# Shuijing725/CrowdNav_Prediction_AttnGraph

Measured on AMD Instinct MI355X. Metric: env-steps/sec (sim+policy fwd) at 20 humans, higher is better.
Workload: dtype f32 (big GEMMs as bf16x3 split-precision MFMA, fp32 accumulate); 1 GPU; BASELINE configs[1]: CrowdSimVarNum-v0, 20 humans, 4096 parallel envs per GPU, HH+HR attention on, policy forward + ORCA sim step + auto-reset per step; envs_per_gpu=4096, humans=20, parallelism=dp1 (envs sharded, no rollout collective), policy_init=orthogonal, torch.manual_seed(425), sampled_actions=True, side_stream_tail=inline, dephase_steps=240

## Files before the change

### crowdnav_prediction_attngraph_amd/_abi.py

```python
import ctypes as C
import os

_PKG = os.path.dirname(os.path.abspath(__file__))
LIB_PATH = os.environ.get("CN_HIP_LIB") or os.path.join(_PKG, "libcrowdnav_hip.so")

CN_MAX_HUMANS = 64
ABI_VERSION = 407
PROF_KERNELS, PROF_SLOT_WORDS = 8, 2048
PROF_KERNEL_IDS = {"env_step": 0, "orca_lane": 1, "hh_fused": 2, "rn_fused": 3, "orca_lp3": 4, "env_pregen": 5, "row_plan": 6, "other": 7}
ENV_KINDS = {"CrowdSimVarNum-v0": 0, "CrowdSimPred-v0": 1, "CrowdSimPredRealGST-v0": 2, "CrowdSimVarNumCollect-v0": 3}
GSTD_MODES = {None: 0, "train": 1, "val": 2, "test": 2}
GSTD_FRAME_ORDER, GSTD_DUPLICATE_ID, GSTD_TOO_MANY_PEDS = 1, 2, 4
INFO_NOTHING, INFO_TIMEOUT, INFO_COLLISION, INFO_REACHGOAL, INFO_DANGER = range(5)


class CnError(RuntimeError):
    pass


class EnvConfig(C.Structure):
    _fields_ = [
        ("human_num", C.c_int32), ("predict_steps", C.c_int32), ("env_kind", C.c_int32),
        ("randomize_attributes", C.c_int32), ("random_goal_changing", C.c_int32),
        ("end_goal_changing", C.c_int32), ("sort_humans", C.c_int32), ("phase", C.c_int32),
# ... 191 lines not shown

class SrnnEdgeGrads(C.Structure):
    _fields_ = [(name, C.c_void_p) for name, _ in SRNN_EDGE_KEYS]


class PpoBatch(C.Structure):
    _fields_ = [(n, C.c_int) for n in ("T", "N", "E", "H", "D")] + [(n, C.c_void_p) for n in PPO_BATCH_TENSORS]


class PpoHyper(C.Structure):
    _fields_ = [("clip_param", C.c_float), ("value_loss_coef", C.c_float), ("entropy_coef", C.c_float), ("use_clipped_value_loss", C.c_int)]


ABI_SYMBOLS = [
    "cn_last_error", "cn_version", "cn_device_count", "cn_env_config_default", "cn_env_create", "cn_env_destroy",
    "cn_env_obs_width", "cn_row_plan_words", "cn_env_set_pregen_budget", "cn_env_set_tail_deferral", "cn_env_launch_tail", "cn_policy_set_post_hh_hook", "cn_env_reset", "cn_env_step", "cn_env_join", "cn_env_get_state", "cn_env_get_human_actions", "cn_env_get_danger_min_dist", "cn_env_get_human_counts", "cn_env_set_case_counters", "cn_env_snapshot_bytes", "cn_env_save", "cn_env_load", "cn_orca_solve",
    "cn_policy_create", "cn_policy_create_sized", "cn_policy_destroy", "cn_policy_set_weights", "cn_policy_act", "cn_policy_get_value",
    "cn_policy_get_taps", "cn_policy_set_gemm_mode", "cn_policy_set_self_attention", "cn_obs_compact_visible", "cn_policy_set_taps", "cn_policy_set_profiling", "cn_policy_get_profile",
    "cn_policy_get_profile_samples", "cn_policy_reset_profile", "cn_prof_set_stamps", "cn_prof_next_step", "cn_hh_block_workspace_bytes", "cn_hh_block_fwd", "cn_rn_seq_workspace_floats", "cn_rn_seq_fwd_workspace_floats", "cn_rn_seq_fwd", "cn_rn_seq_bwd", "cn_rn_seq_workspace_floats_sized", "cn_rn_seq_fwd_workspace_floats_sized", "cn_rn_seq_fwd_sized", "cn_rn_seq_bwd_sized", "cn_gru_seq_fwd_sized", "cn_gru_seq_bwd_sized", "cn_hh_attention_workspace_ints", "cn_hh_attention_fwd", "cn_hh_attention_bwd", "cn_hr_attention_fwd", "cn_hr_attention_bwd", "cn_gru_seq_fwd", "cn_gru_seq_bwd", "cn_embed0_fwd", "cn_embed0_bwd",
    "cn_split_bf16", "cn_split_bf16_padded", "cn_linear_fwd", "cn_linear_fwd_act", "cn_linear_wgrad_splits", "cn_linear_wgrad", "cn_small_mm", "cn_gst_create", "cn_gst_create_horizon", "cn_gst_pred_steps", "cn_gst_destroy", "cn_gst_set_weights", "cn_gst_predict",
    "cn_gst_wrapper_reset", "cn_gst_wrapper_step", "cn_gst_wrapper_set_interval", "cn_gst_wrapper_history_len", "cn_gst_wrapper_save", "cn_gst_wrapper_load", "cn_gae", "cn_adv_stats", "cn_adv_normalize", "cn_episode_stats_update", "cn_eval_state_words", "cn_eval_accumulate",
    "cn_ppo_loss_workspace_doubles", "cn_ppo_loss_fwd", "cn_ppo_loss_bwd", "cn_adam_workspace_doubles", "cn_adam_clip_step",
    "cn_ppo_minibatch_max_rows", "cn_ppo_minibatch_workspace_bytes", "cn_ppo_row_totals", "cn_ppo_minibatch_step",
    "cn_gst_train_workspace_bytes", "cn_gst_train_step", "cn_gst_eval_workspace_bytes", "cn_gst_eval_step",
    "cn_gst_train_workspace_bytes_horizon", "cn_gst_train_step_horizon", "cn_gst_eval_workspace_bytes_horizon", "cn_gst_eval_step_horizon",
    "cn_gst_data_frames_horizon", "cn_gst_data_count_horizon", "cn_gst_data_fill_horizon", "cn_gst_gather_batch_horizon",
    "cn_env_get_visibility", "cn_render_scenes",
    "cn_env_trace_append", "cn_trace_metrics", "cn_render_trajectories",
    "cn_gst_data_frames", "cn_gst_data_count", "cn_gst_data_fill", "cn_gst_gather_batch",
    "cn_srnn_create", "cn_srnn_destroy", "cn_srnn_set_weights", "cn_srnn_act", "cn_srnn_get_value", "cn_srnn_get_taps", "cn_srnn_set_gemm_mode",
    "cn_srnn_seq_workspace_bytes", "cn_srnn_seq_fwd", "cn_srnn_seq_bwd",
# ... 20 lines not shown
                          % (LIB_PATH, L.cn_version(), ABI_VERSION))
        L.cn_env_config_default.argtypes = [C.POINTER(EnvConfig)]
        L.cn_env_config_default.restype = None
        L.cn_env_create.argtypes = [C.POINTER(EnvConfig), i32, i64, i64, C.POINTER(vp)]
        L.cn_env_destroy.argtypes = [vp]
        L.cn_env_obs_width.argtypes = [C.POINTER(EnvConfig)]
        L.cn_env_reset.argtypes = [vp, C.POINTER(Obs), vp]
        L.cn_env_step.argtypes = [vp, vp, C.POINTER(Obs), vp, vp, vp, vp, vp, vp, vp]
        L.cn_env_join.argtypes = [vp, vp]
        L.cn_env_set_pregen_budget.argtypes = [vp, C.c_int64]
        L.cn_env_set_tail_deferral.argtypes = [vp, i32]
        L.cn_env_launch_tail.argtypes = [vp, vp]
        L.cn_policy_set_post_hh_hook.argtypes = [vp, vp, vp]
        L.cn_row_plan_words.restype = C.c_int64
        L.cn_row_plan_words.argtypes = [C.c_int]
        L.cn_env_get_state.argtypes = [vp, vp, vp, vp]
        L.cn_env_get_danger_min_dist.argtypes = [vp, vp, vp]
        L.cn_env_set_case_counters.argtypes = [vp, vp, vp]
        L.cn_env_get_human_counts.argtypes = [vp, vp, vp]
        L.cn_env_get_human_actions.argtypes = [vp, vp, vp]
        L.cn_env_get_visibility.argtypes = [vp, vp, vp]
        L.cn_render_scenes.argtypes = [i32, i32, vp, vp, vp, vp, vp, vp, vp, i32, f32, f32, i32, f32, vp, vp]
        L.cn_env_trace_append.argtypes = [vp, vp, vp, i32, vp, vp, vp, vp, vp]
        L.cn_trace_metrics.argtypes = [i32, i32, i32, vp, vp, vp, f64, f64, vp, vp]
        L.cn_render_trajectories.argtypes = [i32, i32, i32, vp, vp, vp, vp, i32, i32, f32, vp, vp]
        L.cn_env_snapshot_bytes.argtypes = [vp]
        L.cn_env_snapshot_bytes.restype = i64
        L.cn_env_save.argtypes = [vp, vp, vp]
        L.cn_env_load.argtypes = [vp, vp, vp]
        L.cn_orca_solve.argtypes = [i32, i32, vp, vp, f32, i32, f32, f32, vp, vp]
# ... 174 lines not shown
```

### crowdnav_prediction_attngraph_amd/csrc/env_sim.hip

```cpp
#include "common.h"
#include "env_dev.h"
#include "env_profile.h"
#include "det_math.h"
#include "orca.h"
#include "mt19937.h"
#include "episode.h"

#include <hip/hip_ext.h>
#include <cmath>
#include <cstdio>
#include <cstdlib>
#include <cstring>
#include <new>
#include <type_traits>

namespace {

__global__ __launch_bounds__(64) void env_reset_kernel(EnvDev s, cn_obs ob, int with_obs)
{
    const int lane = threadIdx.x;
    const int e = blockIdx.x;
    Rng R{MT_N, false};
    Robot rb{};
    Lane h{};
// ... 833 lines not shown
    b->pregen_ticks = 4000;
    b->lp3_blocks = lp3_grid(num_envs * HM);
    *out = b;
    return CN_OK;
}

extern "C" int cn_env_set_pregen_budget(cn_env_batch *env, int64_t ticks_10ns)
{
    CN_REQUIRE(env && ticks_10ns >= 0, "cn_env_set_pregen_budget: null handle or negative budget");
    env->pregen_ticks = ticks_10ns;
    return CN_OK;
}

extern "C" int64_t cn_row_plan_words(int num_envs) { return num_envs > 0 ? (int64_t)rp_words(num_envs) : 0; }

extern "C" int cn_env_destroy(cn_env_batch *env)
{
    if (!env) return CN_OK;
    (void)hipStreamSynchronize(env->side);
    if (env->side2) { (void)hipStreamSynchronize(env->side2); (void)hipStreamDestroy(env->side2); }
    if (env->ev_pg) (void)hipEventDestroy(env->ev_pg);
    (void)hipEventDestroy(env->ev_state); (void)hipEventDestroy(env->ev_orca); (void)hipEventDestroy(env->ev_pre); (void)hipStreamDestroy(env->side);
    if (env->blob) CN_HIP(hipFree(env->blob));
    delete env;
    return CN_OK;
}

static int check_obs(const cn_obs *obs)
{
    CN_REQUIRE(obs && obs->robot_node && obs->temporal_edges && obs->spatial_edges && obs->detected_human_num,
// ... 217 lines not shown
```

### crowdnav_prediction_attngraph_amd/csrc/orca.h

```cpp
#pragma once
#include "env_dev.h"
#include "det_math.h"

namespace {

struct LpLine { float px, py, dx, dy; };

__device__ __forceinline__ bool wv_any(bool p) { return __ballot(p) != 0ull; }

__device__ __forceinline__ bool lp1_wave(const LpLine &L, uint64_t valid, int i, float ipx, float ipy, float idx, float idy,
                                         float radius, float optx, float opty, bool dirOpt, int lane, float &rx, float &ry)
{
    const float dotProduct = ipx * idx + ipy * idy;
    const float discriminant = dotProduct * dotProduct + radius * radius - (ipx * ipx + ipy * ipy);
    if (discriminant < 0.0f) return false;
    const float sq = sqrtf(discriminant);
    float tLeft = -dotProduct - sq;
    float tRight = -dotProduct + sq;
    const bool mine = lane < i && ((valid >> lane) & 1ull);
    const float denominator = idx * L.dy - idy * L.dx;
    const float numerator = L.dx * (ipy - L.py) - L.dy * (ipx - L.px);
    const bool parallel = fabsf(denominator) <= RVO_EPS;
    const bool pfail = mine && parallel && numerator < 0.0f;
    const float t = numerator / denominator;
// ... 390 lines not shown
    if (plan && (int)blockIdx.x < plan_groups) {
        __builtin_amdgcn_s_setprio(3);
        rowplan::build((int)blockIdx.x, plan_groups, s.E, s.H, rp_workgroups(s.E, s.H), plan_det, plan, *reinterpret_cast<rowplan::Lds *>(s_raw), nullptr, s.plan_arrive);
        return;
    }
    const int blk = (int)blockIdx.x - (plan ? plan_groups : 0);
    typedef typename LaneVec<VW>::f vec;
    const int agent = blk * 64 + threadIdx.x;
    const int H = s.H;
    const bool live_lane = agent < s.E * H;
    const int e = live_lane ? agent / H : (blk * 64) / H, i = live_lane ? agent - e * H : 0;
    const int n = crowd_size(s, e);
    const bool active = live_lane && i < n;
    const cn_env_config &c = s.cfg;
    constexpr int NENV = NB == 8 ? 65 : (NB == 20 ? 10 : 5);
    __shared__ double s_px[128], s_py[128], s_vx[128], s_vy[128], s_rad[128], s_rob[NENV][4];
    const double *hum = s.hum + (size_t)e * 8 * H;
    const size_t ei = (size_t)e * H + i;
    double sgx, sgy, svpref, shared_nd_in;
    int sim_valid_in, sim_n_in = 0;
    float sim_nd_in, sim_r_in, sim_ms_in;
    {
        const int a0 = blk * 64;
        const int e0 = a0 / H, e1 = (min(a0 + 63, s.E * H - 1)) / H;
        const int nrows = (e1 - e0 + 1) * H;
        double st[2][5];
#pragma unroll
        for (int it = 0; it < 2; ++it) {
            const int r = threadIdx.x + 64 * it;
            if (r < nrows) {
                const int ee = e0 + r / H, j = r - (r / H) * H;
                const double *hm = s.hum + (size_t)ee * 8 * H;
                st[it][0] = hm[F_PX * H + j]; st[it][1] = hm[F_PY * H + j]; st[it][2] = hm[F_VX * H + j]; st[it][3] = hm[F_VY * H + j];
                st[it][4] = hm[F_RAD * H + j];
            }
        }
        sgx = hum[F_GX * H + i]; sgy = hum[F_GY * H + i]; svpref = hum[F_VPREF * H + i];
        sim_valid_in = s.sim_valid[ei];
        if (s.sim_n) sim_n_in = s.sim_n[ei];
        sim_nd_in = s.sim_nd[ei]; sim_r_in = s.sim_self_radius[ei]; sim_ms_in = s.sim_self_maxspeed[ei];
        shared_nd_in = s.shared_nd[e];
#pragma unroll
        for (int it = 0; it < 2; ++it) {
            const int r = threadIdx.x + 64 * it;
            if (r < nrows) { s_px[r] = st[it][0]; s_py[r] = st[it][1]; s_vx[r] = st[it][2]; s_vy[r] = st[it][3]; s_rad[r] = st[it][4]; }
        }
        if (c.robot_visible)
            for (int q = threadIdx.x; q <= e1 - e0; q += 64) {
                const double *rb = s.rob + (size_t)(e0 + q) * 8;
                s_rob[q][0] = rb[R_PX]; s_rob[q][1] = rb[R_PY]; s_rob[q][2] = rb[R_VX]; s_rob[q][3] = rb[R_VY];
            }
        __syncthreads();
    }
    const int eq = e - (blk * 64) / H, eb = eq * H;
    const double spx = s_px[eb + i], spy = s_py[eb + i], svx = s_vx[eb + i], svy = s_vy[eb + i], srad = s_rad[eb + i];
    const double safety = c.orca_safety_space;
    const bool rv = c.robot_visible != 0;
    const int n_agents = n + (rv ? 1 : 0);
    float nd = 0.0f, self_r = 0.0f, self_ms = 0.0f;
    if (active) {
        const bool rebuild = !sim_valid_in || (s.sim_n && sim_n_in != n_agents);
        if (rebuild) {
            nd = (float)shared_nd_in;
            self_r = (float)(srad + 0.01 + safety);
            self_ms = (float)svpref;
            if (s.sim_seen)
                for (int j = 0; j < n; ++j) s.sim_seen[ei * H + j] = (float)(s_rad[eb + j] + 0.01 + safety);
            s.sim_nd[ei] = nd; s.sim_self_radius[ei] = self_r; s.sim_self_maxspeed[ei] = self_ms; s.sim_valid[ei] = 1;
            if (s.sim_n) s.sim_n[ei] = (uint8_t)n_agents;
        } else {
            nd = sim_nd_in; self_r = sim_r_in; self_ms = sim_ms_in;
        }
    }
    const float fpx = (float)spx, fpy = (float)spy, fvx = (float)svx, fvy = (float)svy;
    vec key, idx;
    int nn = 0;
#pragma unroll 1
    for (int j = 0; j < NB; ++j) {
        const bool isR = rv && j == n;
        const bool cand = active && ((j < n && j != i) || isR);
        const int lj = j < n ? j : 0;
        const double qx = isR ? s_rob[eq][0] : s_px[eb + lj], qy = isR ? s_rob[eq][1] : s_py[eb + lj];
        const bool coincident = (qx == spx) && (qy == spy);
        const float opx = coincident ? 7.0f : (float)qx, opy = coincident ? 7.0f : (float)qy;
        const float ddx0 = fpx - opx, ddy0 = fpy - opy;
        const float dq = ddx0 * ddx0 + ddy0 * ddy0;
        const bool inrange = cand && dq < nd * nd;
        key[j] = inrange ? dq : INFINITY;
        idx[j] = (float)j;
        nn += inrange ? 1 : 0;
    }
#define ORCA_CE(a, b)                                                                                  \
    {                                                                                                  \
        const float ka0 = key[a], kb0 = key[b], ia0 = idx[a], ib0 = idx[b];                             \
        const bool sw = kb0 < ka0 || (kb0 == ka0 && ib0 < ia0);                                         \
        key[a] = sw ? kb0 : ka0; key[b] = sw ? ka0 : kb0; idx[a] = sw ? ib0 : ia0; idx[b] = sw ? ia0 : ib0; \
    }
    if constexpr (NB == 8) { ORCA_SORTNET_8(ORCA_CE) }
    else if constexpr (NB == 20) { ORCA_SORTNET_20(ORCA_CE) }
    else { static_assert(NB == 32, "sorting networks exist for 8, 20 and 32 slots"); ORCA_SORTNET_32(ORCA_CE) }
#undef ORCA_CE
    int nmax = nn;
    for (int off = 32; off >= 1; off >>= 1) nmax = max(nmax, __shfl_xor(nmax, off, 64));
    nmax = __builtin_amdgcn_readfirstlane(nmax);
    const float invTH = 1.0f / (float)c.orca_time_horizon, invDT = 1.0f / (float)c.time_step;
    float4 *const s_line = reinterpret_cast<float4 *>(s_raw);
    const int tid = threadIdx.x;
#pragma unroll 1
    for (int k = 0; k < nmax; ++k) {
        float o_px = 0.0f, o_py = 0.0f, o_dx = 1.0f, o_dy = 0.0f;
        const int j = (int)idx[k];
        if (k < nn) {
            const bool isR = j == n;
            const int lj = isR ? 0 : j;
            const double qx = isR ? s_rob[eq][0] : s_px[eb + lj], qy = isR ? s_rob[eq][1] : s_py[eb + lj];
            const double qvx = isR ? s_rob[eq][2] : s_vx[eb + lj], qvy = isR ? s_rob[eq][3] : s_vy[eb + lj];
            float orad;
            if (isR) orad = (float)(c.robot_radius + 0.01 + safety);
            else if (s.sim_seen) orad = s.sim_seen[ei * H + lj];
            else orad = (float)(s_rad[eb + lj] + 0.01 + safety);
            const bool coincident = (qx == spx) && (qy == spy);
            const float opx = coincident ? 7.0f : (float)qx, opy = coincident ? 7.0f : (float)qy;
            const float ovx = coincident ? 0.0f : (float)qvx, ovy = coincident ? 0.0f : (float)qvy;
            const float rpx = opx - fpx, rpy = opy - fpy;
            const float rvx = fvx - ovx, rvy = fvy - ovy;
            const float distSq = rpx * rpx + rpy * rpy;
            const float cr = self_r + orad;
            const float crSq = cr * cr;
            const bool collide = !(distSq > crSq);
            const float invT = collide ? invDT : invTH;
            const float wx = rvx - invT * rpx, wy = rvy - invT * rpy;
            const float wLenSq = wx * wx + wy * wy;
            const float dot1 = wx * rpx + wy * rpy;
            const bool circle = collide || (dot1 < 0.0f && dot1 * dot1 > crSq * wLenSq);
            const float sq = sqrtf(circle ? wLenSq : distSq - crSq);
            const float inv = 1.0f / (circle ? sq : distSq);
            const float uwx = wx * inv, uwy = wy * inv;
            const float sc = cr * invT - sq;
            const bool left = rpx * wy - rpy * wx > 0.0f;
            const float lgx = left ? (rpx * sq - rpy * cr) * inv : -((rpx * sq + rpy * cr) * inv);
            const float lgy = left ? (rpx * cr + rpy * sq) * inv : -((-rpx * cr + rpy * sq) * inv);
            const float dot2 = rvx * lgx + rvy * lgy;
            const float ldx = circle ? uwy : lgx, ldy = circle ? -uwx : lgy;
            const float ux = circle ? sc * uwx : dot2 * lgx - rvx, uy = circle ? sc * uwy : dot2 * lgy - rvy;
            o_px = fvx + 0.5f * ux; o_py = fvy + 0.5f * uy; o_dx = ldx; o_dy = ldy;
        }
        s_line[k * 64 + tid] = make_float4(o_px, o_py, o_dx, o_dy);
    }
    double gvx = sgx - spx, gvy = sgy - spy;
    const double speed = sqrt(gvx * gvx + gvy * gvy);
    if (speed > 1.0) { gvx = gvx / speed; gvy = gvy / speed; }
    const float optx = (float)gvx, opty = (float)gvy, radius = self_ms;
    float rx, ry;
    if (optx * optx + opty * opty > radius * radius) {
        const float inv = 1.0f / sqrtf(optx * optx + opty * opty);
        rx = radius * (optx * inv); ry = radius * (opty * inv);
    } else {
        rx = optx; ry = opty;
    }
    unsigned *const s_tl = reinterpret_cast<unsigned *>(s_line + (NB - 1) * 64), *const s_tr = s_tl + 64;
    int *const s_pf = reinterpret_cast<int *>(s_tr + 64), *const s_vl = s_pf + 64;
    auto okey = [](float f) { const unsigned u = __float_as_uint(f); return u ^ ((u >> 31) ? 0xffffffffu : 0x80000000u); };
    auto okey_inv = [](unsigned o) { return __uint_as_float(o ^ ((o >> 31) ? 0x80000000u : 0xffffffffu)); };
    bool failed = false;
    int line_fail = 0;
#pragma unroll 1
    for (int li = 0; li < nmax; ++li) {
        const float4 Li = s_line[li * 64 + tid];
        const float ipx = Li.x, ipy = Li.y, idx_ = Li.z, idy = Li.w;
        const bool viol = li < nn && !failed && idx_ * (ipy - ry) - idy * (ipx - rx) > 0.0f;
        const unsigned long long vm = __ballot(viol);
        if (vm == 0ull) continue;
        const float dotProduct = ipx * idx_ + ipy * idy;
        const float discriminant = dotProduct * dotProduct + radius * radius - (ipx * ipx + ipy * ipy);
        bool ok = !(discriminant < 0.0f);
        const float sq = sqrtf(discriminant);
        float tLeft = -dotProduct - sq, tRight = -dotProduct + sq;
        bool pfail = false;
        const int npairs = __popcll(vm) * li;
        if (npairs > 0) {
            if (viol) {
                const int rank = __builtin_amdgcn_mbcnt_hi((unsigned)(vm >> 32), __builtin_amdgcn_mbcnt_lo((unsigned)vm, 0u));
                s_vl[rank] = tid; s_tl[tid] = okey(tLeft); s_tr[tid] = okey(tRight); s_pf[tid] = 0;
            }
            __syncthreads();
            const unsigned inv20 = ((1u << 20) + (unsigned)li - 1u) / (unsigned)li;
#pragma unroll 1
            for (int p0 = 0; p0 < npairs; p0 += 64) {
                const int p = p0 + tid;
                const bool on = p < npairs;
                const int r = on ? (int)(((unsigned)p * inv20) >> 20) : 0;
                const int lj = on ? p - r * li : 0;
                const int a = s_vl[r];
                const float4 A = s_line[li * 64 + a], B = s_line[lj * 64 + a];
                const float denominator = A.z * B.w - A.w * B.z;
                const float numerator = B.z * (A.y - B.y) - B.w * (A.x - B.x);
                const bool parallel = fabsf(denominator) <= RVO_EPS;
                const float t = numerator / denominator;
                if (on) {
                    if (parallel) { if (numerator < 0.0f) s_pf[a] = 1; }
                    else if (denominator >= 0.0f) atomicMin(&s_tr[a], okey(t));
// ... 141 lines not shown
```

### crowdnav_prediction_attngraph_amd/csrc/row_plan.h

```cpp
#pragma once
#include <stdint.h>

#define RP_MAGIC 0x52504c4e
#define RP_TMAX 1024
#define RP_EMAX 4096
#define RP_HMAX 32
#define RP_HDR 8

__host__ __device__ inline int rp_off_rowoff() { return RP_HDR; }
__host__ __device__ inline int rp_off_tcnt(int E) { return RP_HDR + ((E + 1 + 3) & ~3); }
__host__ __device__ inline int rp_off_items(int E) { return rp_off_tcnt(E) + RP_TMAX; }
__host__ __device__ inline int rp_words(int E) { return rp_off_items(E) + RP_TMAX * 64; }
__host__ __device__ inline int rp_workgroups(int E, int H)
{
    long long g = ((long long)E * H + 15) / 16;
    return g > 256 ? 256 : (g < 1 ? 1 : (int)g);
}
__host__ __device__ inline int rp_groups(int E)
{
    if (E <= 0 || (E & 255)) return 1;
    return E >= 2048 ? 8 : (E >= 1024 ? 4 : (E >= 512 ? 2 : 1));
}

#ifdef __HIPCC__
// ... 42 lines not shown
template <int TBP>
__device__ __forceinline__ bool fill(int H, int T, int TB, int rows, int hist, int cstart, int id_base, int32_t *__restrict__ items, int32_t *__restrict__ tcnt,
                                     Lds &lds, long long *tim)
{
    const int ln = threadIdx.x & 63;
    int load[TBP], cnt[TBP];
    bool own[TBP];
#pragma unroll
    for (int j = 0; j < TBP; ++j) { load[j] = 0; cnt[j] = 0; own[j] = j < TB && ln * TB + j < T; }
    const int base = rows / T, extra = rows - base * T;
    int cap0[TBP];
#pragma unroll
    for (int j = 0; j < TBP; ++j) { const int c0 = base + (ln * TB + j < extra ? 1 : 0); cap0[j] = c0 > 63 ? 63 : c0; }
    bool bad = false;
    int rot = 0;
    for (int v = H; v >= 1; --v) {
        const int m = __builtin_amdgcn_readlane(hist, v);
        if (m == 0) continue;
        const int pos0 = __builtin_amdgcn_readlane(cstart, v);
        RP_A0();
        const unsigned inv = ((1u << 20) + (unsigned)v - 1u) / (unsigned)v;
        int placed = 0;
        constexpr int NPASS = 13;
        const int raise[NPASS] = {0, 0, 1, 2, 3, 4, 6, 8, 12, 16, 24, 32, 63};
        for (int pass = 0; pass < NPASS && placed < m; ++pass) {
            const int left = m - placed;
            const int quota = pass == 0 ? (left + T - 1) / T : 64;
            int c[TBP], lc = 0;
#pragma unroll
            for (int j = 0; j < TBP; ++j) {
                int cap = cap0[j] + raise[pass];
                cap = cap > 63 ? 63 : cap;
                int r = own[j] && load[j] < cap ? (int)(((unsigned)(cap - load[j]) * inv) >> 20) : 0;
                r = r < 63 - cnt[j] ? r : 63 - cnt[j];
                r = r < quota ? r : quota;
                c[j] = r; lc += r;
// ... 28 lines not shown
            placed += fit < left ? fit : left;
            RP_A(10);
        }
        if (placed < m) bad = true;
    }
#pragma unroll
    for (int j = 0; j < TBP; ++j)
        if (own[j]) {
            tcnt[ln * TB + j] = cnt[j];
            items[(size_t)(ln * TB + j) * 64 + cnt[j]] = 0;
            if (load[j] > 63) bad = true;
        }
    return __ballot(bad) == 0ull;
}

__device__ __forceinline__ void build(int g, int G, int E, int H, int NW, const float *__restrict__ det, int32_t *__restrict__ plan, Lds &lds, long long *tim = nullptr,
                                      int32_t *arrive = nullptr)
{
    const int ln = threadIdx.x & 63;
    int32_t *hdr = plan, *row_off = plan + rp_off_rowoff(), *tcnt = plan + rp_off_tcnt(E), *items = plan + rp_off_items(E);
    RP_T(0);
    if (ln == 0) hdr[0] = 0;
    if (H > RP_HMAX || E > RP_EMAX || (E & 3)) return;
    const int CH = ((E + 255) >> 8) << 2;
    int mysum = 0;
    {
        int c[64];
#pragma unroll
        for (int q = 0; q < 16; ++q) {
            float4 d = float4{0.f, 0.f, 0.f, 0.f};
            const int e0 = ln * CH + 4 * q;
            if (4 * q < CH && e0 < E) d = *reinterpret_cast<const float4 *>(det + e0);
            const float dd[4] = {d.x, d.y, d.z, d.w};
#pragma unroll
            for (int u = 0; u < 4; ++u) {
                int r = (int)dd[u];
                r = r < 1 ? 1 : (r > H ? H : r);
                c[4 * q + u] = (4 * q < CH && e0 < E) ? r : 0;
            }
        }
#pragma unroll
        for (int i = 0; i < 64; ++i) mysum += c[i];
        const int incl0 = wave_incl_scan(mysum);
        const int LG = 64 / G;
        if (ln / LG == g || G == 1) {
            int run = incl0 - mysum;
#pragma unroll
            for (int q = 0; q < 16; ++q) {
                int4 o;
                o.x = run; run += c[4 * q]; o.y = run; run += c[4 * q + 1]; o.z = run; run += c[4 * q + 2]; o.w = run; run += c[4 * q + 3];
                if (4 * q < CH && ln * CH + 4 * q < E) *reinterpret_cast<int4 *>(row_off + ln * CH + 4 * q) = o;
            }
        }
        mysum = incl0;
    }
    const int total = __builtin_amdgcn_readlane(mysum, 63);
    if (g == 0 && ln == 0) row_off[E] = total;
    int n = (total + 62 * NW - 1) / (62 * NW);
    n = n < 1 ? 1 : n;
    const int Tall = n * NW;
    int e_base = 0, Eg = E, t0 = 0, T = Tall, grows = total;
    if (G > 1) {
        const int LG = 64 / G;
        const int cum0 = g ? __builtin_amdgcn_readlane(mysum, g * LG - 1) : 0, cum1 = __builtin_amdgcn_readlane(mysum, (g + 1) * LG - 1);
        grows = cum1 - cum0;
        t0 = (int)(((long long)cum0 * Tall + total / 2) / total);
        const int t1 = g == G - 1 ? Tall : (int)(((long long)cum1 * Tall + total / 2) / total);
        T = t1 - t0;
        Eg = E / G; e_base = g * Eg;
    }
    bool ok = T >= 1 && Tall <= RP_TMAX;
    int c[64];
    int hist = 0, cstart = 0;
    if (ok) {
        const int CHg = ((Eg + 255) >> 8) << 2;
#pragma unroll
        for (int q = 0; q < 16; ++q) {
            float4 d = float4{0.f, 0.f, 0.f, 0.f};
            const int e0 = ln * CHg + 4 * q;
            const bool in = 4 * q < CHg && e0 < Eg;
            if (in) d = *reinterpret_cast<const float4 *>(det + e_base + e0);
            const float dd[4] = {d.x, d.y, d.z, d.w};
#pragma unroll
            for (int u = 0; u < 4; ++u) {
                int r = (int)dd[u];
                r = r < 1 ? 1 : (r > H ? H : r);
                c[4 * q + u] = in ? r : 0;
            }
        }
        for (int k = ln; k < (H + 1) * 64; k += 64) lds.tbl[k] = 0;
#pragma unroll
        for (int i = 0; i < 64; ++i)
            if (c[i]) __hip_atomic_fetch_add(&lds.tbl[c[i] * 64 + ln], 1, __ATOMIC_RELAXED, __HIP_MEMORY_SCOPE_WORKGROUP);
        RP_T(1);
        {
            int at = 0;
            for (int v = H; v >= 1; --v) {
                const int mine = lds.tbl[v * 64 + ln];
                const int incl = wave_incl_scan(mine);
                lds.tbl[v * 64 + ln] = at + incl - mine;
                const int m = __builtin_amdgcn_readlane(incl, 63);
                if (ln == v) { hist = m; cstart = at; }
                at += m;
            }
        }
        {
            int pos[64];
#pragma unroll
            for (int i = 0; i < 64; ++i)
                pos[i] = c[i] ? __hip_atomic_fetch_add(&lds.tbl[c[i] * 64 + ln], 1, __ATOMIC_RELAXED, __HIP_MEMORY_SCOPE_WORKGROUP) : 0;
#pragma unroll
            for (int i = 0; i < 64; ++i)
                if (c[i]) lds.ids[pos[i]] = (unsigned short)(ln * CHg + i);
        }
        RP_T(2);
        const int TB = (T + 63) >> 6;
        int32_t *it = items + (size_t)t0 * 64, *tc = tcnt + t0;
        if (TB <= 1) ok = fill<1>(H, T, TB, grows, hist, cstart, e_base, it, tc, lds, tim);
        else if (TB <= 2) ok = fill<2>(H, T, TB, grows, hist, cstart, e_base, it, tc, lds, tim);
        else if (TB <= 4) ok = fill<4>(H, T, TB, grows, hist, cstart, e_base, it, tc, lds, tim);
        else if (TB <= 8) ok = fill<8>(H, T, TB, grows, hist, cstart, e_base, it, tc, lds, tim);
        else ok = fill<16>(H, T, TB, grows, hist, cstart, e_base, it, tc, lds, tim);
    }
    RP_T(3);
    __threadfence();
    if (ln == 0) {
        int32_t *ctr = arrive ? arrive : &hdr[7];
        const int old = G > 1 ? atomicAdd(ctr, ok ? 1 : 0x10001) : (ok ? 0 : 0x10000);
        if ((old & 0xffff) == G - 1) {
// ... 15 lines not shown
```

### include/crowdnav_hip.h

```cpp
#ifndef CROWDNAV_HIP_H
#define CROWDNAV_HIP_H

#include <stddef.h>
#include <stdint.h>

#ifdef __cplusplus
extern "C" {
#endif

typedef enum {
    CN_OK = 0,
    CN_ERR_INVALID = -1,
    CN_ERR_HIP = -2,
    CN_ERR_NO_DEVICE = -3,
    CN_ERR_STATE = -4
} cn_status;

enum { CN_ENV_VARNUM = 0, CN_ENV_PRED = 1, CN_ENV_PRED_GST = 2, CN_ENV_COLLECT = 3 };
enum { CN_PHASE_TRAIN = 0, CN_PHASE_VAL = 1, CN_PHASE_TEST = 2 };
enum { CN_INFO_NOTHING = 0, CN_INFO_TIMEOUT = 1, CN_INFO_COLLISION = 2, CN_INFO_REACHGOAL = 3, CN_INFO_DANGER = 4 };

enum { CN_ROBOT_NETWORK = 0, CN_ROBOT_ORCA = 1, CN_ROBOT_SOCIAL_FORCE = 2 };
enum { CN_KIN_HOLONOMIC = 0, CN_KIN_UNICYCLE = 1 };
enum { CN_HUMANS_ORCA = 0, CN_HUMANS_SOCIAL_FORCE = 1 };
// ... 44 lines not shown
typedef struct cn_policy cn_policy;

#define CN_ABI_VERSION 407
const char *cn_last_error(void);
int cn_version(void);
int cn_device_count(void);

void cn_env_config_default(cn_env_config *cfg);
int cn_env_create(const cn_env_config *cfg, int num_envs, int64_t seed, int64_t first_env_index, cn_env_batch **out);
int cn_env_destroy(cn_env_batch *env);
int cn_env_obs_width(const cn_env_config *cfg);
int cn_env_set_pregen_budget(cn_env_batch *env, int64_t ticks_10ns);
int cn_env_set_tail_deferral(cn_env_batch *env, int enabled);
int cn_env_launch_tail(cn_env_batch *env, void *stream);
int64_t cn_row_plan_words(int num_envs);
int cn_env_reset(cn_env_batch *env, const cn_obs *obs, void *stream);
int cn_env_step(cn_env_batch *env, const float *actions, const cn_obs *obs, float *reward, uint8_t *done, uint8_t *info,
                double *ep_return, int32_t *ep_len, float *not_done, void *stream);
int cn_env_join(cn_env_batch *env, void *stream);
int cn_env_get_state(cn_env_batch *env, double *humans, double *robot, void *stream);
int cn_env_get_human_actions(cn_env_batch *env, float *out, void *stream);
int cn_env_get_danger_min_dist(cn_env_batch *env, double *out, void *stream);
int cn_env_get_human_counts(cn_env_batch *env, int32_t *out, void *stream);
int cn_env_get_visibility(cn_env_batch *env, uint8_t *out, void *stream);
int cn_env_trace_append(cn_env_batch *env, const int64_t *active, const int64_t *index, int cap, float *agents, uint8_t *flags, float *goal,
                        int32_t *length, void *stream);
int cn_env_set_case_counters(cn_env_batch *env, const uint64_t *counters, void *stream);

int64_t cn_env_snapshot_bytes(const cn_env_batch *env);
int cn_env_save(cn_env_batch *env, void *dst, void *stream);
// ... 301 lines not shown
```

Measured before the change: 16.75 million env-steps/s.

## Use float LDS staging, packed-key sort and templated row-plan histogram in ORCA

The ORCA lane kernel now stages neighbour position, velocity and inflated radius as float4/float in shared memory instead of five double arrays. The neighbour filter runs a fully unrolled float pass and falls back to the exact double coincidence check only when some lane sees an equal position. The sorting network now compares packed 64-bit (key, index) values. Per-lane reciprocal tables replace integer divisions in the LP and row-plan loops. The row-plan builder reuses prefetched detection counts, sizes its histogram and hand-out loops to the real chunk count, and unrolls the class scan by eight; a standalone row-plan build entry point is also added. Together these aim to cut LDS traffic, double-precision arithmetic, register pressure and serial scan latency, at the risk of subtle numeric or ordering differences.

Result: faster. 16.95 million env-steps/s (median of 6 runs) (+1.2%).

```diff
diff --git a/crowdnav_prediction_attngraph_amd/_abi.py b/crowdnav_prediction_attngraph_amd/_abi.py
--- a/crowdnav_prediction_attngraph_amd/_abi.py
+++ b/crowdnav_prediction_attngraph_amd/_abi.py
@@ -229,7 +229,7 @@
 
 ABI_SYMBOLS = [
     "cn_last_error", "cn_version", "cn_device_count", "cn_env_config_default", "cn_env_create", "cn_env_destroy",
-    "cn_env_obs_width", "cn_row_plan_words", "cn_env_set_pregen_budget", "cn_env_set_tail_deferral", "cn_env_launch_tail", "cn_policy_set_post_hh_hook", "cn_env_reset", "cn_env_step", "cn_env_join", "cn_env_get_state", "cn_env_get_human_actions", "cn_env_get_danger_min_dist", "cn_env_get_human_counts", "cn_env_set_case_counters", "cn_env_snapshot_bytes", "cn_env_save", "cn_env_load", "cn_orca_solve",
+    "cn_env_obs_width", "cn_row_plan_words", "cn_row_plan_build", "cn_env_set_pregen_budget", "cn_env_set_tail_deferral", "cn_env_launch_tail", "cn_policy_set_post_hh_hook", "cn_env_reset", "cn_env_step", "cn_env_join", "cn_env_get_state", "cn_env_get_human_actions", "cn_env_get_danger_min_dist", "cn_env_get_human_counts", "cn_env_set_case_counters", "cn_env_snapshot_bytes", "cn_env_save", "cn_env_load", "cn_orca_solve",
     "cn_policy_create", "cn_policy_create_sized", "cn_policy_destroy", "cn_policy_set_weights", "cn_policy_act", "cn_policy_get_value",
     "cn_policy_get_taps", "cn_policy_set_gemm_mode", "cn_policy_set_self_attention", "cn_obs_compact_visible", "cn_policy_set_taps", "cn_policy_set_profiling", "cn_policy_get_profile",
     "cn_policy_get_profile_samples", "cn_policy_reset_profile", "cn_prof_set_stamps", "cn_prof_next_step", "cn_hh_block_workspace_bytes", "cn_hh_block_fwd", "cn_rn_seq_workspace_floats", "cn_rn_seq_fwd_workspace_floats", "cn_rn_seq_fwd", "cn_rn_seq_bwd", "cn_rn_seq_workspace_floats_sized", "cn_rn_seq_fwd_workspace_floats_sized", "cn_rn_seq_fwd_sized", "cn_rn_seq_bwd_sized", "cn_gru_seq_fwd_sized", "cn_gru_seq_bwd_sized", "cn_hh_attention_workspace_ints", "cn_hh_attention_fwd", "cn_hh_attention_bwd", "cn_hr_attention_fwd", "cn_hr_attention_bwd", "cn_gru_seq_fwd", "cn_gru_seq_bwd", "cn_embed0_fwd", "cn_embed0_bwd",
@@ -280,6 +280,7 @@
         L.cn_policy_set_post_hh_hook.argtypes = [vp, vp, vp]
         L.cn_row_plan_words.restype = C.c_int64
         L.cn_row_plan_words.argtypes = [C.c_int]
+        L.cn_row_plan_build.argtypes = [i32, i32, vp, vp, vp]
         L.cn_env_get_state.argtypes = [vp, vp, vp, vp]
         L.cn_env_get_danger_min_dist.argtypes = [vp, vp, vp]
         L.cn_env_set_case_counters.argtypes = [vp, vp, vp]
diff --git a/crowdnav_prediction_attngraph_amd/csrc/env_sim.hip b/crowdnav_prediction_attngraph_amd/csrc/env_sim.hip
--- a/crowdnav_prediction_attngraph_amd/csrc/env_sim.hip
+++ b/crowdnav_prediction_attngraph_amd/csrc/env_sim.hip
@@ -871,6 +871,25 @@
 
 extern "C" int64_t cn_row_plan_words(int num_envs) { return num_envs > 0 ? (int64_t)rp_words(num_envs) : 0; }
 
+__global__ __launch_bounds__(64) void row_plan_kernel(int E, int H, const float *det, int32_t *plan)
+{
+    __shared__ rowplan::Lds lds;
+    rowplan::build((int)blockIdx.x, (int)gridDim.x, E, H, rp_workgroups(E, H), det, plan, lds);
+}
+
+extern "C" int cn_row_plan_build(int num_envs, int rows, const float *detected_human_num, int32_t *row_plan, void *stream)
+{
+    if (int rc = cn_require_device()) return rc;
+    CN_REQUIRE(num_envs > 0 && rows >= 1 && detected_human_num && row_plan, "cn_row_plan_build: null argument or empty batch");
+    CN_REQUIRE((((uintptr_t)detected_human_num | (uintptr_t)row_plan) & 15u) == 0, "cn_row_plan_build: both buffers must be 16-byte aligned");
+    hipStream_t st = (hipStream_t)stream;
+    CN_HIP(hipMemsetAsync(row_plan, 0, RP_HDR * sizeof(int32_t), st));
+    if (num_envs > RP_EMAX) return CN_OK;
+    hipLaunchKernelGGL(row_plan_kernel, dim3(rp_groups(num_envs)), dim3(64), 0, st, num_envs, rows, detected_human_num, row_plan);
+    CN_CHECK_LAUNCH();
+    return CN_OK;
+}
+
 extern "C" int cn_env_destroy(cn_env_batch *env)
 {
     if (!env) return CN_OK;
diff --git a/crowdnav_prediction_attngraph_amd/csrc/orca.h b/crowdnav_prediction_attngraph_amd/csrc/orca.h
--- a/crowdnav_prediction_attngraph_amd/csrc/orca.h
+++ b/crowdnav_prediction_attngraph_amd/csrc/orca.h
@@ -1,6 +1,7 @@
 #pragma once
 #include "env_dev.h"
 #include "det_math.h"
+#include <type_traits>
 
 namespace {
 
@@ -428,9 +429,12 @@
     const bool active = live_lane && i < n;
     const cn_env_config &c = s.cfg;
     constexpr int NENV = NB == 8 ? 65 : (NB == 20 ? 10 : 5);
-    __shared__ double s_px[128], s_py[128], s_vx[128], s_vy[128], s_rad[128], s_rob[NENV][4];
+    __shared__ double s_px[128], s_py[128], s_rob[NENV][2];
+    __shared__ float4 s_f4[128], s_frob[NENV];
+    __shared__ float s_fr[128];
     const double *hum = s.hum + (size_t)e * 8 * H;
     const size_t ei = (size_t)e * H + i;
+    const double safety = c.orca_safety_space;
     double sgx, sgy, svpref, shared_nd_in;
     int sim_valid_in, sim_n_in = 0;
     float sim_nd_in, sim_r_in, sim_ms_in;
@@ -457,18 +461,24 @@
 #pragma unroll
         for (int it = 0; it < 2; ++it) {
             const int r = threadIdx.x + 64 * it;
-            if (r < nrows) { s_px[r] = st[it][0]; s_py[r] = st[it][1]; s_vx[r] = st[it][2]; s_vy[r] = st[it][3]; s_rad[r] = st[it][4]; }
+            if (r < nrows) {
+                s_px[r] = st[it][0]; s_py[r] = st[it][1];
+                s_f4[r] = make_float4((float)st[it][0], (float)st[it][1], (float)st[it][2], (float)st[it][3]);
+                s_fr[r] = (float)(st[it][4] + 0.01 + safety);
+            }
         }
         if (c.robot_visible)
             for (int q = threadIdx.x; q <= e1 - e0; q += 64) {
                 const double *rb = s.rob + (size_t)(e0 + q) * 8;
-                s_rob[q][0] = rb[R_PX]; s_rob[q][1] = rb[R_PY]; s_rob[q][2] = rb[R_VX]; s_rob[q][3] = rb[R_VY];
+                const double rx0 = rb[R_PX], ry0 = rb[R_PY], rvx0 = rb[R_VX], rvy0 = rb[R_VY];
+                s_rob[q][0] = rx0; s_rob[q][1] = ry0;
+                s_frob[q] = make_float4((float)rx0, (float)ry0, (float)rvx0, (float)rvy0);
             }
         __syncthreads();
     }
     const int eq = e - (blk * 64) / H, eb = eq * H;
-    const double spx = s_px[eb + i], spy = s_py[eb + i], svx = s_vx[eb + i], svy = s_vy[eb + i], srad = s_rad[eb + i];
-    const double safety = c.orca_safety_space;
+    const double spx = s_px[eb + i], spy = s_py[eb + i];
+    const float4 self4 = s_f4[eb + i];
     const bool rv = c.robot_visible != 0;
     const int n_agents = n + (rv ? 1 : 0);
     float nd = 0.0f, self_r = 0.0f, self_ms = 0.0f;
@@ -476,66 +486,105 @@
         const bool rebuild = !sim_valid_in || (s.sim_n && sim_n_in != n_agents);
         if (rebuild) {
             nd = (float)shared_nd_in;
-            self_r = (float)(srad + 0.01 + safety);
+            self_r = s_fr[eb + i];
             self_ms = (float)svpref;
             if (s.sim_seen)
-                for (int j = 0; j < n; ++j) s.sim_seen[ei * H + j] = (float)(s_rad[eb + j] + 0.01 + safety);
+                for (int j = 0; j < n; ++j) s.sim_seen[ei * H + j] = s_fr[eb + j];
             s.sim_nd[ei] = nd; s.sim_self_radius[ei] = self_r; s.sim_self_maxspeed[ei] = self_ms; s.sim_valid[ei] = 1;
             if (s.sim_n) s.sim_n[ei] = (uint8_t)n_agents;
         } else {
             nd = sim_nd_in; self_r = sim_r_in; self_ms = sim_ms_in;
         }
     }
-    const float fpx = (float)spx, fpy = (float)spy, fvx = (float)svx, fvy = (float)svy;
+    const float fpx = self4.x, fpy = self4.y, fvx = self4.z, fvy = self4.w;
+    float4 rob4 = make_float4(0.0f, 0.0f, 0.0f, 0.0f);
+    if (rv) rob4 = s_frob[eq];
+    const float rob_r = (float)(c.robot_radius + 0.01 + safety);
     vec key, idx;
     int nn = 0;
+    unsigned coin = 0u;
+    {
+        const float ndSq = nd * nd;
+        bool feq = false;
+        auto pass1 = [&](auto with_robot) {
+#pragma unroll
+            for (int j = 0; j < NB; ++j) {
+                float qx = s_f4[eb + j].x, qy = s_f4[eb + j].y;
+                bool cand = active && j < n && j != i;
+                if constexpr (decltype(with_robot)::value) {
+                    const bool isR = j == n;
+                    qx = isR ? rob4.x : qx; qy = isR ? rob4.y : qy;
+                    cand = cand || (active && isR);
+                }
+                feq |= cand & (qx == fpx) & (qy == fpy);
+                const float ddx0 = fpx - qx, ddy0 = fpy - qy;
+                const float dq = ddx0 * ddx0 + ddy0 * ddy0;
+                const bool inrange = cand && dq < ndSq;
+                key[j] = inrange ? dq : INFINITY;
+                nn += inrange ? 1 : 0;
+                if ((j & 3) == 3) __builtin_amdgcn_sched_barrier(0);
+            }
+        };
+        if (rv) pass1(std::true_type{}); else pass1(std::false_type{});
+        if (__ballot(feq) != 0ull) {
+            nn = 0;
 #pragma unroll 1
-    for (int j = 0; j < NB; ++j) {
-        const bool isR = rv && j == n;
-        const bool cand = active && ((j < n && j != i) || isR);
-        const int lj = j < n ? j : 0;
-        const double qx = isR ? s_rob[eq][0] : s_px[eb + lj], qy = isR ? s_rob[eq][1] : s_py[eb + lj];
-        const bool coincident = (qx == spx) && (qy == spy);
-        const float opx = coincident ? 7.0f : (float)qx, opy = coincident ? 7.0f : (float)qy;
-        const float ddx0 = fpx - opx, ddy0 = fpy - opy;
-        const float dq = ddx0 * ddx0 + ddy0 * ddy0;
-        const bool inrange = cand && dq < nd * nd;
-        key[j] = inrange ? dq : INFINITY;
-        idx[j] = (float)j;
-        nn += inrange ? 1 : 0;
-    }
-#define ORCA_CE(a, b)                                                                                  \
-    {                                                                                                  \
-        const float ka0 = key[a], kb0 = key[b], ia0 = idx[a], ib0 = idx[b];                             \
-        const bool sw = kb0 < ka0 || (kb0 == ka0 && ib0 < ia0);                                         \
-        key[a] = sw ? kb0 : ka0; key[b] = sw ? ka0 : kb0; idx[a] = sw ? ib0 : ia0; idx[b] = sw ? ia0 : ib0; \
-    }
-    if constexpr (NB == 8) { ORCA_SORTNET_8(ORCA_CE) }
-    else if constexpr (NB == 20) { ORCA_SORTNET_20(ORCA_CE) }
-    else { static_assert(NB == 32, "sorting networks exist for 8, 20 and 32 slots"); ORCA_SORTNET_32(ORCA_CE) }
+            for (int j = 0; j < NB; ++j) {
+                const bool isR = rv && j == n;
+                const bool cand = active && ((j < n && j != i) || isR);
+                const int lj = j < n ? j : 0;
+                const double qxd = isR ? s_rob[eq][0] : s_px[eb + lj], qyd = isR ? s_rob[eq][1] : s_py[eb + lj];
+                const float qx = isR ? rob4.x : s_f4[eb + lj].x, qy = isR ? rob4.y : s_f4[eb + lj].y;
+                const bool coincident = (qxd == spx) && (qyd == spy);
+                if (cand && coincident) coin |= 1u << j;
+                const float opx = coincident ? 7.0f : qx, opy = coincident ? 7.0f : qy;
+                const float ddx0 = fpx - opx, ddy0 = fpy - opy;
+                const float dq = ddx0 * ddx0 + ddy0 * ddy0;
+                const bool inrange = cand && dq < ndSq;
+                key[j] = inrange ? dq : INFINITY;
+                nn += inrange ? 1 : 0;
+            }
+        }
+    }
+    const bool any_coin = __ballot(coin != 0u) != 0ull;
+    {
+        unsigned long long kv[NB];
+#pragma unroll
+        for (int j = 0; j < NB; ++j) kv[j] = ((unsigned long long)__float_as_uint(key[j]) << 32) | (unsigned)j;
+#define ORCA_CE(a, b)                                                  \
+    {                                                                  \
+        const unsigned long long ka0 = kv[a], kb0 = kv[b];             \
+        const bool sw = kb0 < ka0;                                     \
+        kv[a] = sw ? kb0 : ka0; kv[b] = sw ? ka0 : kb0;                \
+    }
+        if constexpr (NB == 8) { ORCA_SORTNET_8(ORCA_CE) }
+        else if constexpr (NB == 20) { ORCA_SORTNET_20(ORCA_CE) }
+        else { static_assert(NB == 32, "sorting networks exist for 8, 20 and 32 slots"); ORCA_SORTNET_32(ORCA_CE) }
 #undef ORCA_CE
-    int nmax = nn;
-    for (int off = 32; off >= 1; off >>= 1) nmax = max(nmax, __shfl_xor(nmax, off, 64));
-    nmax = __builtin_amdgcn_readfirstlane(nmax);
-    const float invTH = 1.0f / (float)c.orca_time_horizon, invDT = 1.0f / (float)c.time_step;
+#pragma unroll
+        for (int j = 0; j < NB; ++j) idx[j] = __uint_as_float(held((unsigned)kv[j]));
+    }
+    const int nmax = rowplan::wave_max(nn);
+    const float invTH = held(1.0f / (float)c.orca_time_horizon), invDT = held(1.0f / (float)c.time_step);
     float4 *const s_line = reinterpret_cast<float4 *>(s_raw);
     const int tid = threadIdx.x;
 #pragma unroll 1
     for (int k = 0; k < nmax; ++k) {
         float o_px = 0.0f, o_py = 0.0f, o_dx = 1.0f, o_dy = 0.0f;
-        const int j = (int)idx[k];
+        const int j = (int)__float_as_uint(idx[k]);
         if (k < nn) {
             const bool isR = j == n;
             const int lj = isR ? 0 : j;
-            const double qx = isR ? s_rob[eq][0] : s_px[eb + lj], qy = isR ? s_rob[eq][1] : s_py[eb + lj];
-            const double qvx = isR ? s_rob[eq][2] : s_vx[eb + lj], qvy = isR ? s_rob[eq][3] : s_vy[eb + lj];
+            float4 q = s_f4[eb + lj];
             float orad;
-            if (isR) orad = (float)(c.robot_radius + 0.01 + safety);
-            else if (s.sim_seen) orad = s.sim_seen[ei * H + lj];
-            else orad = (float)(s_rad[eb + lj] + 0.01 + safety);
-            const bool coincident = (qx == spx) && (qy == spy);
-            const float opx = coincident ? 7.0f : (float)qx, opy = coincident ? 7.0f : (float)qy;
-            const float ovx = coincident ? 0.0f : (float)qvx, ovy = coincident ? 0.0f : (float)qvy;
+            if (s.sim_seen) orad = s.sim_seen[ei * H + lj];
+            else orad = held(s_fr[eb + lj]);
+            if (rv) { q.x = isR ? rob4.x : q.x; q.y = isR ? rob4.y : q.y; q.z = isR ? rob4.z : q.z; q.w = isR ? rob4.w : q.w; orad = isR ? rob_r : orad; }
+            if (any_coin) {
+                const bool coincident = (coin >> j) & 1u;
+                q.x = coincident ? 7.0f : q.x; q.y = coincident ? 7.0f : q.y; q.z = coincident ? 0.0f : q.z; q.w = coincident ? 0.0f : q.w;
+            }
+            const float opx = q.x, opy = q.y, ovx = q.z, ovy = q.w;
             const float rpx = opx - fpx, rpy = opy - fpy;
             const float rvx = fvx - ovx, rvy = fvy - ovy;
             const float distSq = rpx * rpx + rpy * rpy;
@@ -546,14 +595,15 @@
             const float wx = rvx - invT * rpx, wy = rvy - invT * rpy;
             const float wLenSq = wx * wx + wy * wy;
             const float dot1 = wx * rpx + wy * rpy;
-            const bool circle = collide || (dot1 < 0.0f && dot1 * dot1 > crSq * wLenSq);
+            const bool circle = collide | ((dot1 < 0.0f) & (dot1 * dot1 > crSq * wLenSq));
             const float sq = sqrtf(circle ? wLenSq : distSq - crSq);
             const float inv = 1.0f / (circle ? sq : distSq);
             const float uwx = wx * inv, uwy = wy * inv;
             const float sc = cr * invT - sq;
             const bool left = rpx * wy - rpy * wx > 0.0f;
-            const float lgx = left ? (rpx * sq - rpy * cr) * inv : -((rpx * sq + rpy * cr) * inv);
-            const float lgy = left ? (rpx * cr + rpy * sq) * inv : -((-rpx * cr + rpy * sq) * inv);
+            const float lxl = (rpx * sq - rpy * cr) * inv, lxr = -((rpx * sq + rpy * cr) * inv);
+            const float lyl = (rpx * cr + rpy * sq) * inv, lyr = -((-rpx * cr + rpy * sq) * inv);
+            const float lgx = left ? lxl : lxr, lgy = left ? lyl : lyr;
             const float dot2 = rvx * lgx + rvy * lgy;
             const float ldx = circle ? uwy : lgx, ldy = circle ? -uwx : lgy;
             const float ux = circle ? sc * uwx : dot2 * lgx - rvx, uy = circle ? sc * uwy : dot2 * lgy - rvy;
@@ -578,6 +628,7 @@
     auto okey_inv = [](unsigned o) { return __uint_as_float(o ^ ((o >> 31) ? 0x80000000u : 0xffffffffu)); };
     bool failed = false;
     int line_fail = 0;
+    const unsigned inv20_of_lane = ((1u << 20) + (unsigned)max(tid, 1) - 1u) / (unsigned)max(tid, 1);
 #pragma unroll 1
     for (int li = 0; li < nmax; ++li) {
         const float4 Li = s_line[li * 64 + tid];
@@ -598,7 +649,7 @@
                 s_vl[rank] = tid; s_tl[tid] = okey(tLeft); s_tr[tid] = okey(tRight); s_pf[tid] = 0;
             }
             __syncthreads();
-            const unsigned inv20 = ((1u << 20) + (unsigned)li - 1u) / (unsigned)li;
+            const unsigned inv20 = (unsigned)__builtin_amdgcn_readlane((int)inv20_of_lane, li);
 #pragma unroll 1
             for (int p0 = 0; p0 < npairs; p0 += 64) {
                 const int p = p0 + tid;
diff --git a/crowdnav_prediction_attngraph_amd/csrc/row_plan.h b/crowdnav_prediction_attngraph_amd/csrc/row_plan.h
--- a/crowdnav_prediction_attngraph_amd/csrc/row_plan.h
+++ b/crowdnav_prediction_attngraph_amd/csrc/row_plan.h
@@ -80,12 +80,16 @@
     for (int j = 0; j < TBP; ++j) { const int c0 = base + (ln * TB + j < extra ? 1 : 0); cap0[j] = c0 > 63 ? 63 : c0; }
     bool bad = false;
     int rot = 0;
+    constexpr bool INV_TABLE = TBP <= 4;
+    unsigned inv_of_lane = 0u;
+    if constexpr (INV_TABLE) inv_of_lane = ((1u << 20) + (unsigned)(ln < 1 ? 1 : ln) - 1u) / (unsigned)(ln < 1 ? 1 : ln);
     for (int v = H; v >= 1; --v) {
         const int m = __builtin_amdgcn_readlane(hist, v);
         if (m == 0) continue;
         const int pos0 = __builtin_amdgcn_readlane(cstart, v);
         RP_A0();
-        const unsigned inv = ((1u << 20) + (unsigned)v - 1u) / (unsigned)v;
+        const unsigned inv = INV_TABLE ? (unsigned)__builtin_amdgcn_readlane((int)inv_of_lane, v)
+                                       : ((1u << 20) + (unsigned)v - 1u) / (unsigned)v;
         int placed = 0;
         constexpr int NPASS = 13;
         const int raise[NPASS] = {0, 0, 1, 2, 3, 4, 6, 8, 12, 16, 24, 32, 63};
@@ -144,6 +148,53 @@
     return __ballot(bad) == 0ull;
 }
 
+template <int CHGP>
+__device__ __forceinline__ void size_histogram(const int (&c)[64], int H, Lds &lds)
+{
+    const int ln = threadIdx.x & 63;
+    for (int k = ln; k < (H + 1) * 64; k += 64) lds.tbl[k] = 0;
+#pragma unroll
+    for (int i = 0; i < CHGP; ++i)
+        if (c[i]) __hip_atomic_fetch_add(&lds.tbl[c[i] * 64 + ln], 1, __ATOMIC_RELAXED, __HIP_MEMORY_SCOPE_WORKGROUP);
+}
+__device__ __forceinline__ void class_positions(int H, Lds &lds, int &hist, int &cstart)
+{
+    const int ln = threadIdx.x & 63;
+    int at = 0;
+#pragma unroll
+    for (int b = RP_HMAX - 8; b >= 0; b -= 8) {
+        if (b < H) {
+            int mine[8], incl[8];
+#pragma unroll
+            for (int u = 0; u < 8; ++u) mine[u] = b + 1 + u <= H ? lds.tbl[(b + 1 + u) * 64 + ln] : 0;
+#pragma unroll
+            for (int u = 0; u < 8; ++u) incl[u] = wave_incl_scan(mine[u]);
+#pragma unroll
+            for (int u = 7; u >= 0; --u) {
+                const int v = b + 1 + u;
+                if (v <= H) {
+                    lds.tbl[v * 64 + ln] = at + incl[u] - mine[u];
+                    const int m = __builtin_amdgcn_readlane(incl[u], 63);
+                    if (ln == v) { hist = m; cstart = at; }
+                    at += m;
+                }
+            }
+        }
+    }
+}
+template <int CHGP>
+__device__ __forceinline__ void hand_out_order(const int (&c)[64], int CHg, Lds &lds)
+{
+    const int ln = threadIdx.x & 63;
+    int pos[CHGP];
+#pragma unroll
+    for (int i = 0; i < CHGP; ++i)
+        pos[i] = c[i] ? __hip_atomic_fetch_add(&lds.tbl[c[i] * 64 + ln], 1, __ATOMIC_RELAXED, __HIP_MEMORY_SCOPE_WORKGROUP) : 0;
+#pragma unroll
+    for (int i = 0; i < CHGP; ++i)
+        if (c[i]) lds.ids[pos[i]] = (unsigned short)(ln * CHg + i);
+}
+
 __device__ __forceinline__ void build(int g, int G, int E, int H, int NW, const float *__restrict__ det, int32_t *__restrict__ plan, Lds &lds, long long *tim = nullptr,
                                       int32_t *arrive = nullptr)
 {
@@ -153,14 +204,29 @@
     if (ln == 0) hdr[0] = 0;
     if (H > RP_HMAX || E > RP_EMAX || (E & 3)) return;
     const int CH = ((E + 255) >> 8) << 2;
+    const int Eg = G > 1 ? E / G : E, e_base = G > 1 ? g * Eg : 0;
+    const int CHg = ((Eg + 255) >> 8) << 2;
+    float4 dg[2];
     int mysum = 0;
+    int c[64];
     {
-        int c[64];
+        float4 db[16];
 #pragma unroll
         for (int q = 0; q < 16; ++q) {
-            float4 d = float4{0.f, 0.f, 0.f, 0.f};
+            db[q] = float4{0.f, 0.f, 0.f, 0.f};
             const int e0 = ln * CH + 4 * q;
-            if (4 * q < CH && e0 < E) d = *reinterpret_cast<const float4 *>(det + e0);
+            if (4 * q < CH && e0 < E) db[q] = *reinterpret_cast<const float4 *>(det + e0);
+        }
+#pragma unroll
+        for (int q = 0; q < 2; ++q) {
+            dg[q] = float4{0.f, 0.f, 0.f, 0.f};
+            const int e0 = ln * CHg + 4 * q;
+            if (G > 1 && 4 * q < CHg && e0 < Eg) dg[q] = *reinterpret_cast<const float4 *>(det + e_base + e0);
+        }
+#pragma unroll
+        for (int q = 0; q < 16; ++q) {
+            const float4 d = db[q];
+            const int e0 = ln * CH + 4 * q;
             const float dd[4] = {d.x, d.y, d.z, d.w};
 #pragma unroll
             for (int u = 0; u < 4; ++u) {
@@ -189,7 +255,7 @@
     int n = (total + 62 * NW - 1) / (62 * NW);
     n = n < 1 ? 1 : n;
     const int Tall = n * NW;
-    int e_base = 0, Eg = E, t0 = 0, T = Tall, grows = total;
+    int t0 = 0, T = Tall, grows = total;
     if (G > 1) {
         const int LG = 64 / G;
         const int cum0 = g ? __builtin_amdgcn_readlane(mysum, g * LG - 1) : 0, cum1 = __builtin_amdgcn_readlane(mysum, (g + 1) * LG - 1);
@@ -197,52 +263,33 @@
         t0 = (int)(((long long)cum0 * Tall + total / 2) / total);
         const int t1 = g == G - 1 ? Tall : (int)(((long long)cum1 * Tall + total / 2) / total);
         T = t1 - t0;
-        Eg = E / G; e_base = g * Eg;
     }
     bool ok = T >= 1 && Tall <= RP_TMAX;
-    int c[64];
     int hist = 0, cstart = 0;
     if (ok) {
-        const int CHg = ((Eg + 255) >> 8) << 2;
-#pragma unroll
-        for (int q = 0; q < 16; ++q) {
-            float4 d = float4{0.f, 0.f, 0.f, 0.f};
-            const int e0 = ln * CHg + 4 * q;
-            const bool in = 4 * q < CHg && e0 < Eg;
-            if (in) d = *reinterpret_cast<const float4 *>(det + e_base + e0);
-            const float dd[4] = {d.x, d.y, d.z, d.w};
-#pragma unroll
-            for (int u = 0; u < 4; ++u) {
-                int r = (int)dd[u];
-                r = r < 1 ? 1 : (r > H ? H : r);
-                c[4 * q + u] = in ? r : 0;
-            }
-        }
-        for (int k = ln; k < (H + 1) * 64; k += 64) lds.tbl[k] = 0;
-#pragma unroll
-        for (int i = 0; i < 64; ++i)
-            if (c[i]) __hip_atomic_fetch_add(&lds.tbl[c[i] * 64 + ln], 1, __ATOMIC_RELAXED, __HIP_MEMORY_SCOPE_WORKGROUP);
+        if (G > 1) {
+#pragma unroll
+            for (int q = 0; q < 2; ++q) {
+                const bool in = 4 * q < CHg && ln * CHg + 4 * q < Eg;
+                const float dd[4] = {dg[q].x, dg[q].y, dg[q].z, dg[q].w};
+#pragma unroll
+                for (int u = 0; u < 4; ++u) {
+                    int r = (int)dd[u];
+                    r = r < 1 ? 1 : (r > H ? H : r);
+                    c[4 * q + u] = in ? r : 0;
+                }
+            }
+        }
+        if (CHg <= 8) size_histogram<8>(c, H, lds);
+        else if (CHg <= 16) size_histogram<16>(c, H, lds);
+        else if (CHg <= 32) size_histogram<32>(c, H, lds);
+        else size_histogram<64>(c, H, lds);
         RP_T(1);
-        {
-            int at = 0;
-            for (int v = H; v >= 1; --v) {
-                const int mine = lds.tbl[v * 64 + ln];
-                const int incl = wave_incl_scan(mine);
-                lds.tbl[v * 64 + ln] = at + incl - mine;
-                const int m = __builtin_amdgcn_readlane(incl, 63);
-                if (ln == v) { hist = m; cstart = at; }
-                at += m;
-            }
-        }
-        {
-            int pos[64];
-#pragma unroll
-            for (int i = 0; i < 64; ++i)
-                pos[i] = c[i] ? __hip_atomic_fetch_add(&lds.tbl[c[i] * 64 + ln], 1, __ATOMIC_RELAXED, __HIP_MEMORY_SCOPE_WORKGROUP) : 0;
-#pragma unroll
-            for (int i = 0; i < 64; ++i)
-                if (c[i]) lds.ids[pos[i]] = (unsigned short)(ln * CHg + i);
-        }
+        class_positions(H, lds, hist, cstart);
+        if (CHg <= 8) hand_out_order<8>(c, CHg, lds);
+        else if (CHg <= 16) hand_out_order<16>(c, CHg, lds);
+        else if (CHg <= 32) hand_out_order<32>(c, CHg, lds);
+        else hand_out_order<64>(c, CHg, lds);
         RP_T(2);
         const int TB = (T + 63) >> 6;
         int32_t *it = items + (size_t)t0 * 64, *tc = tcnt + t0;
diff --git a/include/crowdnav_hip.h b/include/crowdnav_hip.h
--- a/include/crowdnav_hip.h
+++ b/include/crowdnav_hip.h
@@ -82,6 +82,7 @@
 int cn_env_set_tail_deferral(cn_env_batch *env, int enabled);
 int cn_env_launch_tail(cn_env_batch *env, void *stream);
 int64_t cn_row_plan_words(int num_envs);
+int cn_row_plan_build(int num_envs, int rows, const float *detected_human_num, int32_t *row_plan, void *stream);
 int cn_env_reset(cn_env_batch *env, const cn_obs *obs, void *stream);
 int cn_env_step(cn_env_batch *env, const float *actions, const cn_obs *obs, float *reward, uint8_t *done, uint8_t *info,
                 double *ep_return, int32_t *ep_len, float *not_done, void *stream);
```
